# pycompression/python-zlib-ng

Hardware: AMD Instinct MI355X
Metric: MB/s compress+decompress, 128 KiB blocks level 6 (higher is better)
Workload: dtype u8

## Files before the change

### python-zlib-ng_amd/csrc/zng_amd.hip

```cpp
#include "za_deflate.hip"
#include "za_inflate.hip"
#include "za_inflate_units.hip"
#include "za_inflate_spans.hip"
#include "za_bgzf.hip"
#include "za_grep.hip"
#include "za_grep_records.hip"
#include "za_tabix.hip"
#include "za_faidx.hip"
#include "za_batch.hip"
#include "za_dict.hip"
#include "za_checksum.hip"
#include "../../include/zng_amd.h"

#include <algorithm>
#include <chrono>
#include <cstdio>
#include <cstdlib>
#include <cstring>
#include <mutex>
#include <string>
#include <thread>
#include <vector>

static_assert(sizeof(zngamd_member) == sizeof(ZaMember), "member layout");
static_assert(sizeof(zngamd_span) == sizeof(ZaSpan) && ZNGAMD_SPAN_PAD == ZA_SPAN_PAD && ZNGAMD_SPAN_CRC == ZA_SPAN_CRC, "span layout");
static_assert(sizeof(zngamd_batch_item) == sizeof(ZaBatchItem) && sizeof(zngamd_batch_result) == sizeof(ZaBatchResult) &&
              ZNGAMD_BATCH_PAD == ZA_BATCH_PAD && ZNGAMD_BATCH_TABLE == ZA_BATCH_TABLE && ZNGAMD_BATCH_OUTFULL == ZA_BATCH_OUTFULL, "batch layout");
static_assert(ZNGAMD_ZDICT_MISMATCH == ZA_ZDICT_MISMATCH, "zdict status");
static_assert(sizeof(zngamd_bgzf_block) == sizeof(ZaBgzfBlock) && sizeof(zngamd_bgzf_slice) == sizeof(ZaBgzfSlice) && ZNGAMD_BGZF_MAX_INPUT == ZA_BGZF_MAX_IN &&
              ZNGAMD_BGZF_SLICE_BLOCK == ZA_SLICE_BLOCK && ZNGAMD_BGZF_SLICE_TABLE == ZA_SLICE_TABLE, "bgzf layout");
static_assert(sizeof(zngamd_bgzf_count_row) == sizeof(ZaBgzfCount) && sizeof(zngamd_bgzf_pos) == sizeof(ZaBgzfPos) && sizeof(zngamd_bgzf_line_range) == 2 * sizeof(ZaBgzfPos) &&
              ZNGAMD_BGZF_SLICE_RANK == ZA_SLICE_RANK && ZNGAMD_BGZF_RANK_END == ZA_RANK_END && ZNGAMD_BGZF_COUNT_LAST == ZA_COUNT_LAST, "bgzf line layout");
static_assert(sizeof(zngamd_bgzf_pattern) == sizeof(ZaGrepPat) && sizeof(zngamd_bgzf_grep_row) == sizeof(ZaGrepRow) && sizeof(ZaGrepRow) == sizeof(ZaBgzfSlice) &&
              sizeof(zngamd_bgzf_grep_totals) == 40 && offsetof(ZaGrepTotals, covered) == offsetof(zngamd_bgzf_grep_totals, covered) && sizeof(ZaGrepTotals) <= 64 &&
              ZNGAMD_BGZF_GREP_INVERT == ZA_GREP_INVERT && ZNGAMD_BGZF_GREP_LINE_START == ZA_GREP_LINE_START && ZNGAMD_BGZF_GREP_FINAL == ZA_GREP_FINAL &&
              ZNGAMD_BGZF_GREP_COUNT_ONLY == ZA_GREP_COUNT_ONLY && ZNGAMD_BGZF_GREP_MAX_PATTERNS == ZA_GREP_MAX_PAT && ZNGAMD_BGZF_GREP_MAX_PATTERN == ZA_GREP_MAX_LEN,
              "bgzf grep layout");
static_assert(sizeof(zngamd_bgzf_grep_records_totals) == sizeof(ZaGrepRecTotals) && sizeof(ZaGrepRecTotals) == 64 &&
              offsetof(ZaGrepRecTotals, covered) == offsetof(zngamd_bgzf_grep_records_totals, covered) && sizeof(ZaGrepTotals) == 56 &&
              ZNGAMD_BGZF_GREP_MAX_RECORD_LINES == ZA_GREP_REC_MAX, "bgzf grep records layout");
static_assert(sizeof(zngamd_tabix_conf) == sizeof(ZaTbxConf) && sizeof(zngamd_tabix_name) == sizeof(ZaTbxName) && sizeof(zngamd_tabix_bin) == sizeof(ZaTbxBin) &&
              sizeof(zngamd_tabix_win) == sizeof(ZaTbxWin) && sizeof(zngamd_tabix_region) == sizeof(ZaTbxRegion) && sizeof(zngamd_tabix_span) == sizeof(ZaTbxSpan) &&
              sizeof(zngamd_tabix_row) == sizeof(ZaTbxRow) && sizeof(zngamd_bgzf_tabix_totals) == 104 && sizeof(ZaTbxState) <= 64 &&
              ZNGAMD_BGZF_TABIX_FINAL == ZA_TBX_FINAL && ZNGAMD_BGZF_FETCH_COUNT_ONLY == ZA_TBX_COUNT_ONLY && ZNGAMD_TABIX_MAX_POS == ZA_TBX_MAX_POS, "bgzf tabix layout");
static_assert(sizeof(zngamd_faidx_carry) == sizeof(ZaFaiCarry) && sizeof(ZaFaiCarry) == 32 && sizeof(zngamd_faidx_row) == sizeof(ZaFaiRow) && sizeof(ZaFaiRow) == 48 &&
              sizeof(zngamd_faidx_span) == sizeof(ZaFaiSpan) && sizeof(ZaFaiSpan) == 40 && sizeof(zngamd_bgzf_faidx_totals) == 104 && sizeof(ZaFaiState) == 88 &&
              ZNGAMD_BGZF_FAIDX_FINAL == ZA_FAI_FINAL && ZNGAMD_FAIDX_SPAN_RC == ZA_FAI_RC && ZNGAMD_FAIDX_MAX_SPAN == ZA_FAI_MAX_SPAN &&
              ZNGAMD_BGZF_SLICE_STALE == ZA_SLICE_STALE && ZNGAMD_FAIDX_OPEN == ZA_FAI_OPEN && ZNGAMD_FAIDX_GAP == ZA_FAI_GAP, "bgzf faidx layout");
static_assert(ZNGAMD_SLOT_STRIDE % 4 == 0 && ZNGAMD_SLOT_STRIDE >= ZA_MAX_UNIT + 32, "slot stride");
static_assert(ZNGAMD_UNIT_MAX == ZA_MAX_UNIT && ZNGAMD_SEG == ZA_SEG, "constants");

#define ZA_CH_STREAMS_PER_CU (ZA_HASH_BITS >= 14 ? 2u : 3u)
static const ZaLevel ZA_LEVELS[10] = {
    {0, 0, ZA_WIN, 0, 0, 0, 0, 0, 3, 0},
    {1, 16, ZA_WIN, 16, 0, 0, 256, 4096, 3, 0}, {2, 16, ZA_WIN, 16, 0, 0, 256, 4096, 3, 0}, {3, 16, ZA_WIN, 16, 0, 0, 256, 4096, 3, 0},
    {2, 16, ZA_WIN, 16, 0, 1, 4096, 32768, 3, 0}, {2, 16, ZA_WIN, 16, 1, 1, 4096, 32768, 3, 0}, {3, 16, ZA_WIN, 16, 1, 1, 4096, 32768, 3, 0},
    {4, 32, ZA_WIN, 258, 1, 1, 4096, 32768, 3, 0}, {8, 64, ZA_WIN, 258, 1, 1, 4096, 32768, 3, 0}, {12, 128, ZA_WIN, 258, 1, 1, 4096, 32768, 3, 0}};

template <typename T> struct DevBuf {
    T *p = nullptr; size_t cap = 0;
    hipError_t ensure(size_t n)
    {
        if (n <= cap) return hipSuccess;
        if (p) { (void)hipFree(p); p = nullptr; cap = 0; }
        size_t want = n * sizeof(T) >= ((size_t)64 << 20) ? n + 64 : n + n / 8 + 64;
        hipError_t e = hipMalloc((void **)&p, want * sizeof(T));
        if (e != hipSuccess) { want = n; e = hipMalloc((void **)&p, want * sizeof(T)); }
        if (e == hipSuccess) cap = want;
        return e;
    }
    void release() { if (p) (void)hipFree(p); p = nullptr; cap = 0; }
};

struct EvPair { hipEvent_t a, b; int cls; };

static thread_local std::string za_tl_err;
struct ZaErrSlot {
    ZaErrSlot &operator=(const char *m) { za_tl_err = m; return *this; }
    ZaErrSlot &operator=(const std::string &m) { za_tl_err = m; return *this; }
    const char *c_str() const { return za_tl_err.c_str(); }
};

struct zngamd_ctx {
    int device = 0;
    hipStream_t own_stream = nullptr, stream = nullptr;
    ZaErrSlot err;
    std::mutex mu;
    uint32_t *d_crc_table = nullptr, *d_x8k = nullptr;
    uint32_t *d_crc_slice4 = nullptr;
    uint32_t chunk_units = 16384;
    DevBuf<uint16_t> links; DevBuf<uint32_t> best, tok, segtok, hist, codes; DevBuf<ZaPlan> plan;
    uint16_t *prev_p = nullptr, *linkb_p = nullptr, *linkc_p = nullptr; uint32_t *tok_p = nullptr;
    bool debug_keep = false, last_kept = false; DevBuf<uint32_t> best_keep, dpcost;
    std::vector<uint32_t> last_ulen_host; bool last_ulen_on_host = false;
    const uint32_t *last_unit_len = nullptr;
    DevBuf<ZaUnit> units; DevBuf<uint32_t> segbits, cidx, status, runs;
    uint32_t last_units = 0; bool last_single_chunk = false;
    std::vector<ZaUnit> last_hu;
    std::vector<ZaUnit> plan_in; std::vector<uint32_t> plan_runs; uint32_t plan_ch = 0;
    std::vector<zngamd_block> blocks_in; std::vector<ZaUnit> blocks_hu; uint64_t blocks_len = 0;
    uint32_t chain_slots = 512;
    uint32_t chain_run = 0;
    DevBuf<uint8_t> st_in, st_out, st_slots, st_aux, hdr; DevBuf<uint32_t> st_len, st_crc; DevBuf<uint64_t> st_off;
    DevBuf<uint64_t> ccand, csurv; DevBuf<ZaChunkRes> cres; DevBuf<ZaChunk> cchunks; DevBuf<uint16_t> out16, ccomp; DevBuf<uint8_t> winbuf;
    DevBuf<uint16_t> uarea; uint32_t uarea_marked = 0;
    DevBuf<ZaCkPart> ck; DevBuf<uint32_t> matchq; DevBuf<ZaCand> cands; DevBuf<ZaMember> members; DevBuf<int32_t> mstatus;
    void *d_small = nullptr;
    uint64_t paths[4] = {0, 0, 0, 0};
    uint64_t indexed_units = 0;
    uint64_t span_stats[2] = {0, 0};
    DevBuf<uint8_t> sp_in, sp_win, sp_out; DevBuf<ZaSpan> sp_tab; DevBuf<int32_t> sp_status;
    DevBuf<uint8_t> bt_out, bt_out2, bt_def; DevBuf<ZaBatchItem> bt_items, bt_items2; DevBuf<ZaBatchResult> bt_res, bt_res2;
    DevBuf<uint32_t> bt_first, bt_ulen, bt_ucrc; DevBuf<uint64_t> bt_uoff, bt_total;
    DevBuf<uint8_t> bt_dict, bt_prime;
    DevBuf<uint8_t> dt_data, dt_dict; DevBuf<uint32_t> dt_hash, dt_freq; DevBuf<uint16_t> dt_shadow;
    DevBuf<ZaBatchItem> dt_items; DevBuf<ZaDictBest> dt_best; DevBuf<ZaDictState> dt_state;
    DevBuf<uint32_t> bg_len; DevBuf<ZaBgzfBlock> bg_table; DevBuf<ZaBgzfSlice> bg_slices; DevBuf<int32_t> bg_sstat; DevBuf<uint8_t> bg_out;
    uint64_t bgzf_stats[3] = {0, 0, 0};
    DevBuf<ZaBgzfCount> bg_rows; DevBuf<ZaBgzfPos> bg_q; DevBuf<uint64_t> bg_pos; DevBuf<int32_t> bg_pstat, bg_pre; DevBuf<uint32_t> bg_rlen;
    DevBuf<uint8_t> gp_par; DevBuf<ulonglong2> gp_bits; DevBuf<ZaGrepTile> gp_tiles; DevBuf<ZaGrepCarry> gp_carry; DevBuf<ZaGrepRow> gp_rows; DevBuf<uint32_t> gp_lens;
    DevBuf<unsigned long long> tb_bits, tb_data, tb_name, tb_bin, tb_key, tb_raise, tb_blk, tb_tot; DevBuf<uint32_t> tb_tcnt, tb_di, tb_lens; DevBuf<uint64_t> tb_tbase;
    DevBuf<ZaTbxLine> tb_lines; DevBuf<ZaTbxName> tb_names; DevBuf<ZaTbxBin> tb_bins; DevBuf<ZaTbxWin> tb_wins;
    DevBuf<uint8_t> tb_par; DevBuf<ZaTbxSpan> tb_spans; DevBuf<ZaTbxRow> tb_rows; DevBuf<uint32_t> tb_srows; DevBuf<int32_t> tb_sstat; DevBuf<uint64_t> tb_sbase;
    std::vector<uint8_t> tb_host;
    DevBuf<unsigned long long> fa_x, fa_bw; DevBuf<uint64_t> fa_start; DevBuf<uint32_t> fa_hline, fa_first, fa_last; DevBuf<ZaFaiRow> fa_rows; DevBuf<ZaFaiSpan> fa_spans;
    DevBuf<unsigned long long> gr_start, gr_sel, gr_len; DevBuf<uint8_t> gr_hit;
    std::vector<uint8_t> gp_host;
    uint8_t *h_stage = nullptr; size_t h_stage_cap = 0;
    uint8_t *h_up = nullptr; size_t h_up_cap = 0;
    uint8_t *h_tab = nullptr; size_t h_tab_cap = 0;
    hipEvent_t ev_up = nullptr, ev_tab = nullptr; bool up_busy = false, tab_busy = false;
    hipEvent_t ev_copy[2] = {nullptr, nullptr};
    bool prof = false; std::vector<EvPair> evs; std::vector<hipEvent_t> pool;
    double ms[ZNGAMD_K_COUNT] = {0}; uint64_t launches[ZNGAMD_K_COUNT] = {0};
};

#define HIPCHK(ctx, call) do { hipError_t e_ = (call); if (e_ != hipSuccess) { \
    (ctx)->err = std::string(#call) + ": " + hipGetErrorString(e_); return ZNGAMD_E_HIP; } } while (0)

static int fail(zngamd_ctx *c, int code, const char *msg) { c->err = msg; return code; }
#define ZA_ABI_GUARD catch (const std::bad_alloc &) { return ZNGAMD_MEM_ERROR; } catch (...) { return ZNGAMD_E_ARG; }


static bool trace_on() { static const bool on = getenv("ZNGAMD_TRACE") != nullptr; return on; }
struct PhaseClock {
    zngamd_ctx *c; const char *name; std::chrono::steady_clock::time_point t;
    PhaseClock(zngamd_ctx *c_, const char *n) : c(c_), name(n) { if (trace_on()) t = std::chrono::steady_clock::now(); }
    ~PhaseClock()
    {
        if (!trace_on()) return;
        if (c) (void)hipStreamSynchronize(c->stream);
        fprintf(stderr, "zng_amd trace: %-34s %9.3f ms\n", name, std::chrono::duration<double, std::milli>(std::chrono::steady_clock::now() - t).count());
    }
};

static hipEvent_t ev_get(zngamd_ctx *c)
{
    if (!c->pool.empty()) { hipEvent_t e = c->pool.back(); c->pool.pop_back(); return e; }
    hipEvent_t e; (void)hipEventCreate(&e); return e;
}
struct ProfScope {
    zngamd_ctx *c; int cls; hipEvent_t a = nullptr;
    ProfScope(zngamd_ctx *c_, int cls_) : c(c_), cls(cls_) { if (c->prof) { a = ev_get(c); (void)hipEventRecord(a, c->stream); } }
    ~ProfScope() { if (c->prof) { hipEvent_t b = ev_get(c); (void)hipEventRecord(b, c->stream); c->evs.push_back({a, b, cls}); } }
};
static void prof_collect(zngamd_ctx *c)
{
    for (auto &e : c->evs) {
        float t = 0; (void)hipEventSynchronize(e.b);
        if (hipEventElapsedTime(&t, e.a, e.b) == hipSuccess) { c->ms[e.cls] += t; c->launches[e.cls]++; }
        c->pool.push_back(e.a); c->pool.push_back(e.b);
    }
    c->evs.clear();
}

extern "C" {

const char *zngamd_version(void) { return "zng_amd 0.6 (gfx950)"; }
int zngamd_abi(void) { return ZNGAMD_ABI; }
int zngamd_kernel_class_count(void) { return ZNGAMD_K_COUNT; }

int zngamd_device_count(void)
try {
    int n = 0;
    if (hipGetDeviceCount(&n) != hipSuccess) return 0;
    return n;
} ZA_ABI_GUARD

int zngamd_ctx_create(int device, zngamd_ctx **out)
try {
    if (!out) return ZNGAMD_E_ARG;
    *out = nullptr;
    int n = 0;
    if (hipGetDeviceCount(&n) != hipSuccess || n <= 0 || device < 0 || device >= n) return ZNGAMD_E_HIP;
    if (hipSetDevice(device) != hipSuccess) return ZNGAMD_E_HIP;
    zngamd_ctx *c = new zngamd_ctx();
    c->device = device;
    if (hipStreamCreateWithFlags(&c->own_stream, hipStreamNonBlocking) != hipSuccess) { delete c; return ZNGAMD_E_HIP; }
    c->stream = c->own_stream;
    if (const char *e = getenv("ZNGAMD_CHUNK_UNITS")) { long v = atol(e); if (v >= 1 && v <= (1 << 20)) c->chunk_units = (uint32_t)v; }
    if (const char *e = getenv("ZNGAMD_CHAIN_RUN")) { long v = atol(e); if (v >= 1 && v <= (1 << 20)) c->chain_run = (uint32_t)v; }
    { int cus = 0; if (hipDeviceGetAttribute(&cus, hipDeviceAttributeMultiprocessorCount, device) == hipSuccess && cus > 0) c->chain_slots = (uint32_t)cus * ZA_CH_STREAMS_PER_CU; }
    uint32_t tab[256], x8k[64];
    for (uint32_t i = 0; i < 256; i++) { uint32_t v = i; for (int k = 0; k < 8; k++) v = (v & 1) ? (0xEDB88320u ^ (v >> 1)) : (v >> 1); tab[i] = v; }
    {
        uint32_t xs = 0x80000000u, sq = 0x00800000u;
        for (int i = 0; i < 11; i++) sq = za_multmodp(sq, sq);
        for (int k = 0; k < 64; k++) { x8k[k] = xs; xs = za_multmodp(xs, sq); }
    }
    if (hipMalloc((void **)&c->d_crc_table, sizeof tab) != hipSuccess || hipMalloc((void **)&c->d_x8k, sizeof x8k) != hipSuccess ||
        hipMalloc(&c->d_small, 256) != hipSuccess ||
        hipMemcpy(c->d_crc_table, tab, sizeof tab, hipMemcpyHostToDevice) != hipSuccess ||
        hipMemcpy(c->d_x8k, x8k, sizeof x8k, hipMemcpyHostToDevice) != hipSuccess) {
        zngamd_ctx_destroy(c); return ZNGAMD_E_HIP;
    }
    {
        std::vector<uint32_t> s4(ZA_CK_TABS);
        for (int i = 0; i < 256; i++) s4[i] = tab[i];
        for (int t = 1; t < 4; t++) for (int i = 0; i < 256; i++) s4[256 * t + i] = (s4[256 * (t - 1) + i] >> 8) ^ tab[s4[256 * (t - 1) + i] & 0xFF];
        uint32_t x32 = 0x00800000u;
        for (int i = 0; i < 5; i++) x32 = za_multmodp(x32, x32);
        uint32_t xs = 0x80000000u;
        for (int k = 0; k < 128; k++) { s4[1152 + k] = xs; xs = za_multmodp(xs, x32); }
        const uint32_t x2016 = s4[1152 + 63];
        for (int k = 0; k < 8; k++) for (uint32_t v = 0; v < 16; v++) s4[1024 + 16 * k + v] = za_multmodp(x2016, v << (4 * k));
        {
            uint32_t xt = 0x80000000u;
            for (int t = 0; t <= 512; t++) { s4[ZA_CK_XT + t] = xt; xt = za_multmodp(xt, 0x00800000u); }
            for (int j = 0; j < 4; j++) {
                const uint32_t step = s4[ZA_CK_XT + (64 << j)];
                uint32_t xk = 0x80000000u;
                for (int k = 0; k < 256; k++) { s4[ZA_CK_XS + 256 * j + k] = xk; xk = za_multmodp(xk, step); }
            }
        }
        if (hipMalloc((void **)&c->d_crc_slice4, s4.size() * 4) != hipSuccess ||
            hipMemcpy(c->d_crc_slice4, s4.data(), s4.size() * 4, hipMemcpyHostToDevice) != hipSuccess) {
            zngamd_ctx_destroy(c); return ZNGAMD_E_HIP;
        }
    }
    *out = c;
    return ZNGAMD_OK;
} ZA_ABI_GUARD

void zngamd_ctx_destroy(zngamd_ctx *c)
{
    if (!c) return;
    (void)hipSetDevice(c->device);
    if (c->stream) (void)hipStreamSynchronize(c->stream);
    prof_collect(c);
    for (auto e : c->pool) (void)hipEventDestroy(e);
    c->links.release(); c->best_keep.release(); c->dpcost.release(); c->hdr.release(); c->best.release(); c->tok.release(); c->segtok.release(); c->hist.release(); c->codes.release();
    c->plan.release(); c->units.release(); c->segbits.release(); c->cidx.release(); c->status.release();
    c->st_in.release(); c->st_out.release(); c->st_slots.release(); c->st_aux.release(); c->st_len.release(); c->st_crc.release();
    c->ccand.release(); c->csurv.release(); c->cres.release(); c->cchunks.release(); c->out16.release(); c->ccomp.release(); c->winbuf.release(); c->uarea.release();
    c->st_off.release(); c->runs.release(); c->ck.release(); c->matchq.release(); c->cands.release(); c->members.release(); c->mstatus.release();
    c->sp_in.release(); c->sp_win.release(); c->sp_out.release(); c->sp_tab.release(); c->sp_status.release();
    c->bt_out.release(); c->bt_out2.release(); c->bt_def.release(); c->bt_items.release(); c->bt_items2.release(); c->bt_res.release(); c->bt_res2.release();
    c->bt_first.release(); c->bt_ulen.release(); c->bt_ucrc.release(); c->bt_uoff.release(); c->bt_total.release();
    c->bt_dict.release(); c->bt_prime.release();
    c->dt_data.release(); c->dt_dict.release(); c->dt_hash.release(); c->dt_freq.release(); c->dt_shadow.release();
    c->dt_items.release(); c->dt_best.release(); c->dt_state.release();
    c->bg_len.release(); c->bg_table.release(); c->bg_slices.release(); c->bg_sstat.release(); c->bg_out.release();
    c->bg_rows.release(); c->bg_q.release(); c->bg_pos.release(); c->bg_pstat.release(); c->bg_pre.release(); c->bg_rlen.release();
    c->tb_bits.release(); c->tb_data.release(); c->tb_name.release(); c->tb_bin.release(); c->tb_key.release(); c->tb_raise.release(); c->tb_blk.release();
    c->tb_tot.release(); c->tb_tcnt.release(); c->tb_di.release(); c->tb_lens.release(); c->tb_tbase.release(); c->tb_lines.release(); c->tb_names.release();
    c->tb_bins.release(); c->tb_wins.release(); c->tb_par.release(); c->tb_spans.release(); c->tb_rows.release(); c->tb_srows.release(); c->tb_sstat.release(); c->tb_sbase.release();
    c->fa_x.release(); c->fa_bw.release(); c->fa_start.release(); c->fa_hline.release(); c->fa_first.release(); c->fa_last.release(); c->fa_rows.release(); c->fa_spans.release();
    c->gp_par.release(); c->gp_bits.release(); c->gp_tiles.release(); c->gp_carry.release(); c->gp_rows.release(); c->gp_lens.release();
    c->gr_start.release(); c->gr_sel.release(); c->gr_len.release(); c->gr_hit.release();
    if (c->h_stage) (void)hipHostFree(c->h_stage);
    if (c->h_up) (void)hipHostFree(c->h_up);
    if (c->h_tab) (void)hipHostFree(c->h_tab);
    if (c->ev_up) (void)hipEventDestroy(c->ev_up);
    if (c->ev_tab) (void)hipEventDestroy(c->ev_tab);
    for (auto &e : c->ev_copy) if (e) (void)hipEventDestroy(e);
    if (c->d_crc_table) (void)hipFree(c->d_crc_table);
    if (c->d_x8k) (void)hipFree(c->d_x8k);
    if (c->d_crc_slice4) (void)hipFree(c->d_crc_slice4);
    if (c->d_small) (void)hipFree(c->d_small);
    if (c->own_stream) (void)hipStreamDestroy(c->own_stream);
    delete c;
}

const char *zngamd_last_error(zngamd_ctx *c) { return c ? c->err.c_str() : "no context"; }

int zngamd_set_stream(zngamd_ctx *c, void *s)
try {
    if (!c) return ZNGAMD_E_ARG;
    (void)hipStreamSynchronize(c->stream);
    c->stream = s ? (hipStream_t)s : c->own_stream;
    return ZNGAMD_OK;
} ZA_ABI_GUARD

int zngamd_sync(zngamd_ctx *c)
try {
    if (!c) return ZNGAMD_E_ARG;
    HIPCHK(c, hipStreamSynchronize(c->stream));
    prof_collect(c);
    return ZNGAMD_OK;
} ZA_ABI_GUARD

int zngamd_dmalloc(zngamd_ctx *c, size_t bytes, void **dptr)
try {
    if (!c || !dptr) return ZNGAMD_E_ARG;
    HIPCHK(c, hipSetDevice(c->device));
    HIPCHK(c, hipMalloc(dptr, bytes ? bytes : 1));
    return ZNGAMD_OK;
} ZA_ABI_GUARD
int zngamd_dfree(zngamd_ctx *c, void *dptr) { if (!c) return ZNGAMD_E_ARG; HIPCHK(c, hipFree(dptr)); return ZNGAMD_OK; }
int zngamd_h2d(zngamd_ctx *c, void *dst, const void *src, size_t bytes)
try {
    if (!c) return ZNGAMD_E_ARG;
    if (bytes) { HIPCHK(c, hipMemcpyAsync(dst, src, bytes, hipMemcpyHostToDevice, c->stream)); HIPCHK(c, hipStreamSynchronize(c->stream)); }
    return ZNGAMD_OK;
} ZA_ABI_GUARD

int zngamd_d2h(zngamd_ctx *c, void *dst, const void *src, size_t bytes)
try {
    if (!c) return ZNGAMD_E_ARG;
    if (bytes) { HIPCHK(c, hipMemcpyAsync(dst, src, bytes, hipMemcpyDeviceToHost, c->stream)); HIPCHK(c, hipStreamSynchronize(c->stream)); }
    return ZNGAMD_OK;
} ZA_ABI_GUARD

int zngamd_d2d(zngamd_ctx *c, void *dst, const void *src, size_t bytes)
try {
    if (!c) return ZNGAMD_E_ARG;
    HIPCHK(c, hipSetDevice(c->device));
    if (bytes) HIPCHK(c, hipMemcpyAsync(dst, src, bytes, hipMemcpyDeviceToDevice, c->stream));
    return ZNGAMD_OK;
} ZA_ABI_GUARD

int zngamd_dmemset(zngamd_ctx *c, void *dst, int value, size_t bytes)
try {
    if (!c) return ZNGAMD_E_ARG;
    HIPCHK(c, hipSetDevice(c->device));
    if (bytes) HIPCHK(c, hipMemsetAsync(dst, value, bytes, c->stream));
    return ZNGAMD_OK;
} ZA_ABI_GUARD

int zngamd_mem_info(zngamd_ctx *c, uint64_t *free_bytes, uint64_t *total_bytes)
try {
    if (!c || !free_bytes || !total_bytes) return ZNGAMD_E_ARG;
    HIPCHK(c, hipSetDevice(c->device));
    size_t f = 0, t = 0;
    HIPCHK(c, hipMemGetInfo(&f, &t));
    *free_bytes = f; *total_bytes = t;
    return ZNGAMD_OK;
} ZA_ABI_GUARD

int zngamd_decode_paths(zngamd_ctx *c, uint64_t *members, int reset)
try {
    if (!c || !members) return ZNGAMD_E_ARG;
    std::lock_guard<std::mutex> g(c->mu);
    for (int i = 0; i < ZNGAMD_PATH_COUNT; i++) { members[i] = c->paths[i]; if (reset) c->paths[i] = 0; }
    return ZNGAMD_OK;
// ... 49 lines not shown
        for (uint64_t k = ZA_MAX_UNIT; k; k >>= 1) { if (k & 1) xp = za_multmodp(sq, xp); sq = za_multmodp(sq, sq); }
        for (uint64_t i = 0; i < nspan; i++) {
            if (parts[i].len == ZA_MAX_UNIT) crc = za_multmodp(xp, crc) ^ parts[i].crc;
            else crc = zngamd_crc32_combine(crc, parts[i].crc, parts[i].len);
        }
        *crc_io = crc;
    }
    if (adler_io) {
        uint64_t A = *adler_io & 0xFFFF, B = (*adler_io >> 16) & 0xFFFF;
        for (uint64_t i = 0; i < nspan; i++) {
            B = (B + (uint64_t)(parts[i].len % 65521u) * A + parts[i].b) % 65521u;
            A = (A + parts[i].a) % 65521u;
        }
        *adler_io = (uint32_t)((B << 16) | A);
    }
}

static int checksum_dev(zngamd_ctx *c, const uint8_t *d, uint64_t n, uint32_t *crc_io, uint32_t *adler_io)
{
    if (n == 0) return ZNGAMD_OK;
    PhaseClock pc(c, "checksum of a device buffer");
    std::vector<ZaCkPart> parts;
    const int r = checksum_launch(c, d, n, crc_io != nullptr, adler_io != nullptr, parts);
    if (r) return r;
    HIPCHK(c, hipStreamSynchronize(c->stream));
    checksum_fold(parts, crc_io, adler_io);
    return ZNGAMD_OK;
}

static int pinned_ensure(zngamd_ctx *c, uint8_t **p, size_t *cap, size_t bytes)
{
    if (bytes <= *cap) return ZNGAMD_OK;
    if (*p) (void)hipHostFree(*p);
    *p = nullptr; *cap = 0;
    const size_t want = bytes + bytes / 4 + 4096;
    HIPCHK(c, hipHostMalloc((void **)p, want, hipHostMallocDefault));
    *cap = want;
    return ZNGAMD_OK;
}

#define ZNGAMD_SMALL_UP (1u << 20)
static int stage_in(zngamd_ctx *c, const uint8_t *in, uint64_t n, uint64_t pad_front = 0)
{
    PhaseClock pc(c, "stage_in (host -> device)");
    HIPCHK(c, hipSetDevice(c->device));
    HIPCHK(c, c->st_in.ensure(pad_front + n + 64));
    if (n <= ZNGAMD_SMALL_UP) {
        if (!c->ev_up) HIPCHK(c, hipEventCreateWithFlags(&c->ev_up, hipEventDisableTiming));
        if (c->up_busy) { HIPCHK(c, hipEventSynchronize(c->ev_up)); c->up_busy = false; }
        const int r = pinned_ensure(c, &c->h_up, &c->h_up_cap, n + 64);
        if (r) return r;
        if (n) memcpy(c->h_up, in, n);
        memset(c->h_up + n, 0, 64);
        HIPCHK(c, hipMemcpyAsync(c->st_in.p + pad_front, c->h_up, n + 64, hipMemcpyHostToDevice, c->stream));
        HIPCHK(c, hipEventRecord(c->ev_up, c->stream));
        c->up_busy = true;
        return ZNGAMD_OK;
    }
    if (n) HIPCHK(c, hipMemcpyAsync(c->st_in.p + pad_front, in, n, hipMemcpyHostToDevice, c->stream));
    HIPCHK(c, hipMemsetAsync(c->st_in.p + pad_front + n, 0, 64, c->stream));
    return ZNGAMD_OK;
}

int zngamd_crc32_dev(zngamd_ctx *c, uint32_t crc, const void *dbuf, size_t len, uint32_t *out)
try {
    if (!c || !out) return ZNGAMD_E_ARG;
    std::lock_guard<std::mutex> g(c->mu);
    HIPCHK(c, hipSetDevice(c->device));
    uint32_t v = crc;
    int r = checksum_dev(c, (const uint8_t *)dbuf, len, &v, nullptr);
    *out = v;
    return r;
} ZA_ABI_GUARD

int zngamd_crc32(zngamd_ctx *c, uint32_t crc, const uint8_t *buf, size_t len, uint32_t *out)
try {
    if (!c || !out || (!buf && len)) return ZNGAMD_E_ARG;
    std::lock_guard<std::mutex> g(c->mu);
    int r = stage_in(c, buf, len);
    if (r) return r;
    uint32_t v = crc;
    r = checksum_dev(c, c->st_in.p, len, &v, nullptr);
    *out = v;
    return r;
} ZA_ABI_GUARD

int zngamd_adler32(zngamd_ctx *c, uint32_t adler, const uint8_t *buf, size_t len, uint32_t *out)
try {
    if (!c || !out || (!buf && len)) return ZNGAMD_E_ARG;
    std::lock_guard<std::mutex> g(c->mu);
    int r = stage_in(c, buf, len);
    if (r) return r;
    uint32_t v = ((((adler >> 16) & 0xFFFFu) % 65521u) << 16) | ((adler & 0xFFFFu) % 65521u);
    r = checksum_dev(c, c->st_in.p, len, nullptr, &v);
    *out = v;
    return r;
} ZA_ABI_GUARD

int zngamd_level_ok(int level) { return level >= -1 && level <= 9; }

static int strategy_of(const zngamd_block *blocks, uint32_t n_blocks) { return n_blocks ? ZNGAMD_STRATEGY_OF(blocks[0].flags) : ZNGAMD_STRATEGY_DEFAULT; }

static uint32_t unit_size_of(const zngamd_block &b) { return (b.flags & ZNGAMD_FLAG_UNITS16K) ? ZA_SMALL_UNIT : (uint32_t)ZA_MAX_UNIT; }
static uint32_t units_of(const zngamd_block &b) { const uint64_t U = unit_size_of(b); return b.len == 0 ? 1u : (uint32_t)(((uint64_t)b.len + U - 1) / U); }

uint32_t zngamd_count_units(const zngamd_block *blocks, uint32_t n_blocks)
{
    uint64_t t = 0;
    for (uint32_t i = 0; i < n_blocks; i++) t += units_of(blocks[i]);
    return t > 0xFFFFFFFFull ? 0xFFFFFFFFu : (uint32_t)t;
}

static int build_units(zngamd_ctx *c, const zngamd_block *blocks, uint32_t n_blocks, uint64_t in_len, std::vector<ZaUnit> &hu)
{
    hu.clear();
    for (uint32_t b = 0; b < n_blocks; b++) {
        const zngamd_block &B = blocks[b];
        if (B.dict_len > ZA_WIN || B.dict_len > B.off || B.off + B.len > in_len) return fail(c, ZNGAMD_E_ARG, "block outside the input buffer");
        const uint32_t nu = units_of(B);
        const uint64_t U = unit_size_of(B);
        for (uint32_t k = 0; k < nu; k++) {
            ZaUnit u;
            const uint64_t rel = (uint64_t)k * U;
            u.in_off = B.off + rel;
            u.in_len = (uint32_t)std::min<uint64_t>(U, B.len - rel);
            u.dict_len = (uint32_t)std::min<uint64_t>(ZA_WIN, (uint64_t)B.dict_len + rel);
            u.flags = (B.flags & (ZNGAMD_FLAG_FLATHDR | ZNGAMD_FLAG_SEG2K)) | ((k == nu - 1) ? (B.flags & ZNGAMD_FLAG_FINAL) : 0u);
            u.flags |= (uint32_t)za_seg_shift_for(u.in_len, u.flags) << 8;
            u.block = b;
            if (!hu.empty()) {
                const ZaUnit &pv = hu.back();
                if (u.dict_len == ZA_WIN && pv.in_len >= ZA_WIN && (pv.in_len & 3u) == 0u && pv.in_off + pv.in_len == u.in_off) u.flags |= ZA_FLAG_CARRY;
            }
            hu.push_back(u);
        }
    }
    return ZNGAMD_OK;
}

struct PackedDst { uint8_t *d_dst = nullptr; uint64_t cap = 0; uint64_t *d_unit_off = nullptr;
                   uint64_t *d_total = nullptr; uint32_t *d_status = nullptr; };
static int deflate_units_dev(zngamd_ctx *c, const uint8_t *d_in, uint64_t in_len, const std::vector<ZaUnit> &hu, int level,
                             uint8_t *d_slots, uint32_t *d_unit_len, uint32_t *d_unit_crc, int max_dist = ZA_WIN,
                             const PackedDst *packed = nullptr, int strategy = ZNGAMD_STRATEGY_DEFAULT)
{
    if (level == -1) level = 6;
    if (level < 0 || level > 9) return fail(c, ZNGAMD_STREAM_ERROR, "Bad compression level");
    if (strategy < ZNGAMD_STRATEGY_DEFAULT || strategy > ZNGAMD_STRATEGY_FIXED) return fail(c, ZNGAMD_STREAM_ERROR, "Bad compression strategy");
    const bool runs_only = level > 0 && (strategy == ZNGAMD_STRATEGY_HUFFMAN_ONLY || strategy == ZNGAMD_STRATEGY_RLE);
    const bool search = level > 0 && !runs_only;
    const uint32_t n = (uint32_t)hu.size();
    if (n == 0) return ZNGAMD_OK;
    HIPCHK(c, hipSetDevice(c->device));
    uint32_t ch = std::min(n, c->chunk_units);
    const size_t ntab = ZA_LEVELS[level].use_c ? 3 : 2;
    if (search) {
        const size_t held = c->links.cap * 2 + c->best.cap * 4 + c->tok.cap * 4 + c->best_keep.cap * 4;
        size_t free_b = 0, total_b = 0;
        if (ch > 64 && hipMemGetInfo(&free_b, &total_b) == hipSuccess) {
            auto need = [&](uint32_t k) { return (size_t)k * (ntab * ZA_PREV_STRIDE * 2 + ZA_BEST_STRIDE * 4 + (c->debug_keep ? (ZA_BEST_STRIDE + ZA_TOK_STRIDE) * 4 : 0) + 8192); };
            while (ch > 64 && need(ch) > held && need(ch) - held > free_b - free_b / 16) ch = (ch + 1) / 2;
        }
    }
    HIPCHK(c, c->units.ensure(n)); HIPCHK(c, c->segbits.ensure((size_t)n * ZA_SEGB_STRIDE)); HIPCHK(c, c->cidx.ensure((size_t)n * ZA_CIDX_STRIDE)); HIPCHK(c, c->status.ensure(n));
    if (runs_only) {
        const size_t held = c->links.cap * 2 + (c->debug_keep ? c->tok.cap * 4 : 0);
        size_t free_b = 0, total_b = 0;
        if (ch > 64 && hipMemGetInfo(&free_b, &total_b) == hipSuccess) {
            auto need = [&](uint32_t k) { return (size_t)k * (ZA_TOK_STRIDE * 4 + 8192); };
            while (ch > 64 && need(ch) > held && need(ch) - held > free_b - free_b / 16) ch = (ch + 1) / 2;
        }
        if (c->debug_keep) { HIPCHK(c, c->tok.ensure((size_t)ch * ZA_TOK_STRIDE)); c->tok_p = c->tok.p; }
        else { HIPCHK(c, c->links.ensure((size_t)ch * ZA_TOK_STRIDE * 2)); c->tok_p = (uint32_t *)c->links.p; }
    }
    if (search) {
        const size_t tab = (size_t)ch * ZA_PREV_STRIDE + 8;
        HIPCHK(c, c->links.ensure(ntab * tab)); HIPCHK(c, c->best.ensure((size_t)ch * ZA_BEST_STRIDE));
        c->prev_p = c->links.p; c->linkb_p = c->links.p + tab; c->linkc_p = ntab > 2 ? c->links.p + 2 * tab : nullptr;
        if (ZA_LEVELS[level].dp) HIPCHK(c, c->dpcost.ensure((size_t)ch * ZA_DP_COSTS));
        if (c->debug_keep) {
            HIPCHK(c, c->best_keep.ensure((size_t)ch * ZA_BEST_STRIDE));
            HIPCHK(c, c->tok.ensure((size_t)ch * ZA_TOK_STRIDE));
            c->tok_p = c->tok.p;
        } else {
            static_assert(2 * ZA_PREV_STRIDE * 2 >= ZA_TOK_STRIDE * 4, "token words fit two link tables");
            c->tok_p = (uint32_t *)c->links.p;
        }
    }
    HIPCHK(c, c->segtok.ensure((size_t)ch * ZA_MAX_SEGS)); HIPCHK(c, c->hist.ensure((size_t)ch * ZA_HIST_STRIDE));
    HIPCHK(c, c->codes.ensure((size_t)ch * ZA_CODE_STRIDE)); HIPCHK(c, c->plan.ensure(ch));
    uint64_t *d_run_total = (uint64_t *)((uint8_t *)c->d_small + 224);
    uint64_t *d_offs = nullptr;
    if (packed) {
        HIPCHK(c, c->hdr.ensure((size_t)ch * ZA_HDR_STRIDE));
        d_offs = packed->d_unit_off;
        if (!d_offs) { HIPCHK(c, c->st_off.ensure(n)); d_offs = c->st_off.p; }
        if (packed->d_total) d_run_total = packed->d_total;
    }
    uint32_t *d_status = (packed && packed->d_status) ? packed->d_status : c->status.p;
    const bool same_plan = c->plan_ch == ch && c->plan_in.size() == hu.size() && c->last_hu.size() == hu.size() &&
                           memcmp(c->plan_in.data(), hu.data(), hu.size() * sizeof(ZaUnit)) == 0;
    if (!same_plan) {
        c->plan_in.clear(); c->plan_ch = 0; c->last_hu.clear();
        std::vector<ZaUnit> hv(hu);
        std::vector<uint32_t> run_start;
        for (uint32_t c0 = 0; c0 < n; c0 += ch) {
            const uint32_t m = std::min(ch, n - c0);
            const uint32_t L = c->chain_run ? c->chain_run : std::min<uint32_t>(8u, std::max<uint32_t>(1u, m / (2u * c->chain_slots)));
            const uint32_t Ls = c->chain_run ? c->chain_run : std::max<uint32_t>(1u, L / 4u);
            const uint32_t big_end = c->chain_run ? m : (uint32_t)((uint64_t)m * 4 / 5 / L * L);
            uint32_t next_cut = 0;
            for (uint32_t i = 0; i < m; i++) {
                ZaUnit &u = hv[c0 + i];
                const bool cut = i == next_cut || !(u.flags & ZA_FLAG_CARRY);
                if (cut) { u.flags |= ZA_FLAG_RUNHEAD; run_start.push_back(i); next_cut = i + (i < big_end ? L : Ls); }
            }
            run_start.push_back(m);
        }
        HIPCHK(c, c->runs.ensure(run_start.size()));
        if (n <= 4096) {
            const size_t rb = run_start.size() * 4, ub = (size_t)n * sizeof(ZaUnit);
            if (!c->ev_tab) HIPCHK(c, hipEventCreateWithFlags(&c->ev_tab, hipEventDisableTiming));
            if (c->tab_busy) { HIPCHK(c, hipEventSynchronize(c->ev_tab)); c->tab_busy = false; }
            const int rp = pinned_ensure(c, &c->h_tab, &c->h_tab_cap, rb + ub);
            if (rp) return rp;
            memcpy(c->h_tab, hv.data(), ub);
            memcpy(c->h_tab + ub, run_start.data(), rb);
            HIPCHK(c, hipMemcpyAsync(c->units.p, c->h_tab, ub, hipMemcpyHostToDevice, c->stream));
            HIPCHK(c, hipMemcpyAsync(c->runs.p, c->h_tab + ub, rb, hipMemcpyHostToDevice, c->stream));
            HIPCHK(c, hipEventRecord(c->ev_tab, c->stream));
            c->tab_busy = true;
        } else {
        HIPCHK(c, hipMemcpyAsync(c->runs.p, run_start.data(), run_start.size() * 4, hipMemcpyHostToDevice, c->stream));
        HIPCHK(c, hipMemcpyAsync(c->units.p, hv.data(), (size_t)n * sizeof(ZaUnit), hipMemcpyHostToDevice, c->stream));
        HIPCHK(c, hipStreamSynchronize(c->stream));
        }
        c->last_hu.swap(hv);
        c->plan_runs.swap(run_start);
        c->plan_in = hu; c->plan_ch = ch;
    }
    const std::vector<uint32_t> &run_start = c->plan_runs;
    ZaLevel L = ZA_LEVELS[level];
    L.max_dist = (max_dist < 1 || max_dist > ZA_WIN) ? ZA_WIN : max_dist;
    if (strategy == ZNGAMD_STRATEGY_FILTERED) L.min_len = 6;
    const int fixed_only = strategy == ZNGAMD_STRATEGY_FIXED ? 1 : 0;
    L.fixed_cost = fixed_only;
    size_t run_pos = 0;
    for (uint32_t c0 = 0; c0 < n; c0 += ch) {
        const uint32_t m = std::min(ch, n - c0);
        const ZaUnit *du = c->units.p + c0;
        uint32_t nruns = 0;
        while (run_start[run_pos + nruns] != m) nruns++;
        const uint32_t *d_runs = c->runs.p + run_pos;
        run_pos += nruns + 1;
        if (runs_only) {
            ProfScope ps(c, ZNGAMD_K_PARSE);
            if (strategy == ZNGAMD_STRATEGY_RLE)
                hipLaunchKernelGGL(za_k_parse_rle<true>, dim3(m), dim3(64), 0, c->stream, d_in, du, c->tok_p, c->segtok.p, c->hist.p,
                                   d_unit_crc + c0, c->d_crc_table, c->d_x8k);
            else
                hipLaunchKernelGGL(za_k_parse_rle<false>, dim3(m), dim3(64), 0, c->stream, d_in, du, c->tok_p, c->segtok.p, c->hist.p,
                                   d_unit_crc + c0, c->d_crc_table, c->d_x8k);
        } else if (search) {
            { ProfScope ps(c, ZNGAMD_K_CHAINS);
              hipLaunchKernelGGL(za_k_chains<ZA_TABLE_A>, dim3(nruns), dim3(256), 0, c->stream, d_in, du, d_runs, c->prev_p, L.dp ? c->dpcost.p : (uint32_t *)nullptr);
              hipLaunchKernelGGL(za_k_chains<ZA_TABLE_B>, dim3(nruns), dim3(256), 0, c->stream, d_in, du, d_runs, c->linkb_p, (uint32_t *)nullptr);
              if (L.use_c) hipLaunchKernelGGL(za_k_chains<ZA_TABLE_C>, dim3(nruns), dim3(256), 0, c->stream, d_in, du, d_runs, c->linkc_p, (uint32_t *)nullptr); }
            { ProfScope ps(c, ZNGAMD_K_SEARCH);
#define ZA_LAUNCH_SEARCH(...) hipLaunchKernelGGL((za_k_search<__VA_ARGS__>), dim3(nruns), dim3(ZA_SEARCH_THREADS), 0, c->stream, d_in, in_len, du, d_runs, \
                                                 c->prev_p, c->linkb_p, L.use_c ? c->linkc_p : c->linkb_p, c->best.p, c->dpcost.p, L)
              if (L.cap > 16) { if (L.use_c) ZA_LAUNCH_SEARCH(true, 0, true); else ZA_LAUNCH_SEARCH(true, 0, false); }
              else if (L.chain == 1) { if (L.use_c) ZA_LAUNCH_SEARCH(false, 1, true); else ZA_LAUNCH_SEARCH(false, 1, false); }
              else if (L.chain == 2) { if (L.use_c) ZA_LAUNCH_SEARCH(false, 2, true); else ZA_LAUNCH_SEARCH(false, 2, false); }
              else if (L.chain == 3) { if (L.use_c) ZA_LAUNCH_SEARCH(false, 3, true); else ZA_LAUNCH_SEARCH(false, 3, false); }
              else { if (L.use_c) ZA_LAUNCH_SEARCH(false, 0, true); else ZA_LAUNCH_SEARCH(false, 0, false); }
#undef ZA_LAUNCH_SEARCH
            }
            if (L.dp) {
                if (c->debug_keep) HIPCHK(c, hipMemcpyAsync(c->best_keep.p, c->best.p, (size_t)m * ZA_BEST_STRIDE * 4, hipMemcpyDeviceToDevice, c->stream));
                ProfScope ps(c, ZNGAMD_K_OPTPARSE);
                if (L.cap > 16 || !ZA_STATS_FOLD) hipLaunchKernelGGL(za_k_dpstats, dim3(m), dim3(256), 0, c->stream, du, c->best.p, c->dpcost.p);
                hipLaunchKernelGGL(za_k_optparse, dim3(m), dim3(64), 0, c->stream, du, c->best.p, c->dpcost.p, c->tok_p, L);
            }
            { ProfScope ps(c, ZNGAMD_K_PARSE);
              if (L.min_len > ZA_MIN_MATCH)
                  hipLaunchKernelGGL(za_k_parse<true>, dim3(m), dim3(64), 0, c->stream, du, c->best.p, c->tok_p, c->segtok.p, c->hist.p,
                                     d_unit_crc + c0, c->d_crc_table, c->d_x8k, L);
              else
                  hipLaunchKernelGGL(za_k_parse<false>, dim3(m), dim3(64), 0, c->stream, du, c->best.p, c->tok_p, c->segtok.p, c->hist.p,
                                     d_unit_crc + c0, c->d_crc_table, c->d_x8k, L); }
        } else {
            ProfScope ps(c, ZNGAMD_K_PARSE);
            hipLaunchKernelGGL(za_k_unit_crc, dim3(m), dim3(64), 0, c->stream, d_in, du, d_unit_crc + c0, c->d_crc_table, c->d_x8k);
        }
        if (packed) {
            { ProfScope ps(c, ZNGAMD_K_PLAN);
              hipLaunchKernelGGL(za_k_plan, dim3(m), dim3(64), 0, c->stream, du, c->hist.p, c->codes.p, c->plan.p,
                                 (uint8_t *)nullptr, 0u, level, c->hdr.p, d_unit_len + c0, fixed_only); }
            { ProfScope ps(c, ZNGAMD_K_GATHER);
              hipLaunchKernelGGL(za_k_offsets, dim3(1), dim3(m <= 64 ? 64 : 1024), 0, c->stream, d_unit_len + c0, m, 0u, 0ull, d_offs + c0, d_run_total,
                                 (const ZaUnit *)nullptr, c0 ? (const uint64_t *)d_run_total : (const uint64_t *)nullptr, 1); }
            { ProfScope ps(c, ZNGAMD_K_PACK);
              hipLaunchKernelGGL(za_k_pack, dim3(m), dim3(64), 0, c->stream, d_in, du, c->tok_p, c->segtok.p, c->codes.p, c->plan.p,
                                 c->segbits.p + (size_t)c0 * ZA_SEGB_STRIDE, c->cidx.p + (size_t)c0 * ZA_CIDX_STRIDE, packed->d_dst,
                                 0u, d_unit_len + c0, d_status + c0, (const uint64_t *)(d_offs + c0), packed->cap, (const uint8_t *)c->hdr.p); }
        } else {
        { ProfScope ps(c, ZNGAMD_K_PLAN);
          hipLaunchKernelGGL(za_k_plan, dim3(m), dim3(64), 0, c->stream, du, c->hist.p, c->codes.p, c->plan.p,
                             d_slots + (size_t)c0 * ZNGAMD_SLOT_STRIDE, (uint32_t)ZNGAMD_SLOT_STRIDE, level, (uint8_t *)nullptr, (uint32_t *)nullptr, fixed_only); }
        { ProfScope ps(c, ZNGAMD_K_PACK);
          hipLaunchKernelGGL(za_k_pack, dim3(m), dim3(64), 0, c->stream, d_in, du, c->tok_p, c->segtok.p, c->codes.p, c->plan.p,
                             c->segbits.p + (size_t)c0 * ZA_SEGB_STRIDE, c->cidx.p + (size_t)c0 * ZA_CIDX_STRIDE, d_slots + (size_t)c0 * ZNGAMD_SLOT_STRIDE,
                             (uint32_t)ZNGAMD_SLOT_STRIDE, d_unit_len + c0, c->status.p + c0, (const uint64_t *)nullptr, 0ull, (const uint8_t *)nullptr); }
        }
        HIPCHK(c, hipGetLastError());
    }
    c->last_units = n; c->last_single_chunk = (n <= ch); c->last_kept = c->debug_keep; c->last_unit_len = d_unit_len; c->last_ulen_on_host = false;
    return ZNGAMD_OK;
}

int zngamd_deflate_blocks_dev(zngamd_ctx *c, const void *d_in, uint64_t in_len, const zngamd_block *blocks, uint32_t n_blocks,
                              int level, void *d_slots, uint32_t *d_unit_len, uint32_t *d_unit_crc, uint32_t *h_unit_block)
try {
    if (!c || (!blocks && n_blocks) || !d_slots || !d_unit_len || !d_unit_crc) return ZNGAMD_E_ARG;
    std::lock_guard<std::mutex> g(c->mu);
    int r = ZNGAMD_OK;
    if (!(n_blocks && c->blocks_in.size() == n_blocks && c->blocks_len == in_len &&
          memcmp(c->blocks_in.data(), blocks, (size_t)n_blocks * sizeof(zngamd_block)) == 0)) {
        c->blocks_in.clear();
        r = build_units(c, blocks, n_blocks, in_len, c->blocks_hu);
        if (r) return r;
        c->blocks_in.assign(blocks, blocks + n_blocks); c->blocks_len = in_len;
    }
    const std::vector<ZaUnit> &hu = c->blocks_hu;
    if (h_unit_block) for (size_t i = 0; i < hu.size(); i++) h_unit_block[i] = hu[i].block;
    r = deflate_units_dev(c, (const uint8_t *)d_in, in_len, hu, level, (uint8_t *)d_slots, d_unit_len, d_unit_crc, ZA_WIN, nullptr,
                          strategy_of(blocks, n_blocks));
    if (r) return r;
    HIPCHK(c, hipStreamSynchronize(c->stream));
    prof_collect(c);
    return ZNGAMD_OK;
} ZA_ABI_GUARD

int zngamd_deflate_blocks_packed_dev(zngamd_ctx *c, const void *d_in, uint64_t in_len, const zngamd_block *blocks, uint32_t n_blocks,
                                     int level, void *d_out, uint64_t out_cap, uint32_t *d_unit_len, uint32_t *d_unit_crc,
                                     uint64_t *d_unit_off, uint64_t *total_bytes)
try {
    if (!c || (!blocks && n_blocks) || !d_out || !d_unit_len || !d_unit_crc || !total_bytes) return ZNGAMD_E_ARG;
    std::lock_guard<std::mutex> g(c->mu);
    int r = ZNGAMD_OK;
    if (!(n_blocks && c->blocks_in.size() == n_blocks && c->blocks_len == in_len &&
          memcmp(c->blocks_in.data(), blocks, (size_t)n_blocks * sizeof(zngamd_block)) == 0)) {
        c->blocks_in.clear();
        r = build_units(c, blocks, n_blocks, in_len, c->blocks_hu);
        if (r) return r;
        c->blocks_in.assign(blocks, blocks + n_blocks); c->blocks_len = in_len;
    }
    const std::vector<ZaUnit> &hu = c->blocks_hu;
    *total_bytes = 0;
    if (hu.empty()) return ZNGAMD_OK;
    PackedDst pd; pd.d_dst = (uint8_t *)d_out; pd.cap = out_cap; pd.d_unit_off = d_unit_off;
    r = deflate_units_dev(c, (const uint8_t *)d_in, in_len, hu, level, nullptr, d_unit_len, d_unit_crc, ZA_WIN, &pd, strategy_of(blocks, n_blocks));
    if (r) return r;
    const uint64_t *d_run_total = (const uint64_t *)((const uint8_t *)c->d_small + 224);
    std::vector<uint32_t> st(hu.size());
    HIPCHK(c, hipMemcpyAsync(total_bytes, d_run_total, 8, hipMemcpyDeviceToHost, c->stream));
    HIPCHK(c, hipMemcpyAsync(st.data(), c->status.p, st.size() * 4ull, hipMemcpyDeviceToHost, c->stream));
    HIPCHK(c, hipStreamSynchronize(c->stream));
// ... 3596 lines not shown
```

Measured before the change: 56730.

## Size chunks by free memory share and taper chain run lengths by slot count

```diff
diff --git a/python-zlib-ng_amd/csrc/zng_amd.hip b/python-zlib-ng_amd/csrc/zng_amd.hip
--- a/python-zlib-ng_amd/csrc/zng_amd.hip
+++ b/python-zlib-ng_amd/csrc/zng_amd.hip
@@ -51,6 +51,7 @@
 static_assert(ZNGAMD_UNIT_MAX == ZA_MAX_UNIT && ZNGAMD_SEG == ZA_SEG, "constants");
 
 #define ZA_CH_STREAMS_PER_CU (ZA_HASH_BITS >= 14 ? 2u : 3u)
+#define ZA_WS_SHARE_DIV 4u
 static const ZaLevel ZA_LEVELS[10] = {
     {0, 0, ZA_WIN, 0, 0, 0, 0, 0, 3, 0},
     {1, 16, ZA_WIN, 16, 0, 0, 256, 4096, 3, 0}, {2, 16, ZA_WIN, 16, 0, 0, 256, 4096, 3, 0}, {3, 16, ZA_WIN, 16, 0, 0, 256, 4096, 3, 0},
@@ -88,7 +89,7 @@
     std::mutex mu;
     uint32_t *d_crc_table = nullptr, *d_x8k = nullptr;
     uint32_t *d_crc_slice4 = nullptr;
-    uint32_t chunk_units = 16384;
+    uint32_t chunk_units = 0;
     DevBuf<uint16_t> links; DevBuf<uint32_t> best, tok, segtok, hist, codes; DevBuf<ZaPlan> plan;
     uint16_t *prev_p = nullptr, *linkb_p = nullptr, *linkc_p = nullptr; uint32_t *tok_p = nullptr;
     bool debug_keep = false, last_kept = false; DevBuf<uint32_t> best_keep, dpcost;
@@ -100,6 +101,7 @@
     std::vector<ZaUnit> plan_in; std::vector<uint32_t> plan_runs; uint32_t plan_ch = 0;
     std::vector<zngamd_block> blocks_in; std::vector<ZaUnit> blocks_hu; uint64_t blocks_len = 0;
     uint32_t chain_slots = 512;
+    uint32_t search_slots = 256;
     uint32_t chain_run = 0;
     DevBuf<uint8_t> st_in, st_out, st_slots, st_aux, hdr; DevBuf<uint32_t> st_len, st_crc; DevBuf<uint64_t> st_off;
     DevBuf<uint64_t> ccand, csurv; DevBuf<ZaChunkRes> cres; DevBuf<ZaChunk> cchunks; DevBuf<uint16_t> out16, ccomp; DevBuf<uint8_t> winbuf;
@@ -200,7 +202,8 @@
     c->stream = c->own_stream;
     if (const char *e = getenv("ZNGAMD_CHUNK_UNITS")) { long v = atol(e); if (v >= 1 && v <= (1 << 20)) c->chunk_units = (uint32_t)v; }
     if (const char *e = getenv("ZNGAMD_CHAIN_RUN")) { long v = atol(e); if (v >= 1 && v <= (1 << 20)) c->chain_run = (uint32_t)v; }
-    { int cus = 0; if (hipDeviceGetAttribute(&cus, hipDeviceAttributeMultiprocessorCount, device) == hipSuccess && cus > 0) c->chain_slots = (uint32_t)cus * ZA_CH_STREAMS_PER_CU; }
+    { int cus = 0; if (hipDeviceGetAttribute(&cus, hipDeviceAttributeMultiprocessorCount, device) == hipSuccess && cus > 0) { c->chain_slots = (uint32_t)cus * ZA_CH_STREAMS_PER_CU; c->search_slots = (uint32_t)cus; } }
+    if (const char *e = getenv("ZNGAMD_CHAIN_SLOTS")) { long v = atol(e); if (v >= 1 && v <= (1 << 20)) { c->chain_slots = (uint32_t)v; c->search_slots = std::max<uint32_t>(1u, (uint32_t)v / ZA_CH_STREAMS_PER_CU); } }
     uint32_t tab[256], x8k[64];
     for (uint32_t i = 0; i < 256; i++) { uint32_t v = i; for (int k = 0; k < 8; k++) v = (v & 1) ? (0xEDB88320u ^ (v >> 1)) : (v >> 1); tab[i] = v; }
     {
@@ -556,24 +559,21 @@
     const uint32_t n = (uint32_t)hu.size();
     if (n == 0) return ZNGAMD_OK;
     HIPCHK(c, hipSetDevice(c->device));
-    uint32_t ch = std::min(n, c->chunk_units);
+    uint32_t ch = c->chunk_units ? std::min(n, c->chunk_units) : n;
     const size_t ntab = ZA_LEVELS[level].use_c ? 3 : 2;
-    if (search) {
-        const size_t held = c->links.cap * 2 + c->best.cap * 4 + c->tok.cap * 4 + c->best_keep.cap * 4;
+    auto fit_set = [&](size_t per_unit, size_t held) {
         size_t free_b = 0, total_b = 0;
-        if (ch > 64 && hipMemGetInfo(&free_b, &total_b) == hipSuccess) {
-            auto need = [&](uint32_t k) { return (size_t)k * (ntab * ZA_PREV_STRIDE * 2 + ZA_BEST_STRIDE * 4 + (c->debug_keep ? (ZA_BEST_STRIDE + ZA_TOK_STRIDE) * 4 : 0) + 8192); };
-            while (ch > 64 && need(ch) > held && need(ch) - held > free_b - free_b / 16) ch = (ch + 1) / 2;
-        }
-    }
+        if (ch <= 64 || hipMemGetInfo(&free_b, &total_b) != hipSuccess) return;
+        auto need = [&](uint32_t k) { return (size_t)k * per_unit; };
+        while (ch > 64 && need(ch) > held && need(ch) - held > free_b - free_b / 16) ch = (ch + 1) / 2;
+        if (!c->chunk_units) while (ch > 64 && need(ch) > (free_b + held) / ZA_WS_SHARE_DIV) ch = (ch + 1) / 2;
+    };
+    if (search)
+        fit_set(ntab * ZA_PREV_STRIDE * 2 + ZA_BEST_STRIDE * 4 + (c->debug_keep ? (ZA_BEST_STRIDE + ZA_TOK_STRIDE) * 4 : 0) + 8192,
+                c->links.cap * 2 + c->best.cap * 4 + c->tok.cap * 4 + c->best_keep.cap * 4);
     HIPCHK(c, c->units.ensure(n)); HIPCHK(c, c->segbits.ensure((size_t)n * ZA_SEGB_STRIDE)); HIPCHK(c, c->cidx.ensure((size_t)n * ZA_CIDX_STRIDE)); HIPCHK(c, c->status.ensure(n));
     if (runs_only) {
-        const size_t held = c->links.cap * 2 + (c->debug_keep ? c->tok.cap * 4 : 0);
-        size_t free_b = 0, total_b = 0;
-        if (ch > 64 && hipMemGetInfo(&free_b, &total_b) == hipSuccess) {
-            auto need = [&](uint32_t k) { return (size_t)k * (ZA_TOK_STRIDE * 4 + 8192); };
-            while (ch > 64 && need(ch) > held && need(ch) - held > free_b - free_b / 16) ch = (ch + 1) / 2;
-        }
+        fit_set(ZA_TOK_STRIDE * 4 + 8192, c->links.cap * 2 + (c->debug_keep ? c->tok.cap * 4 : 0));
         if (c->debug_keep) { HIPCHK(c, c->tok.ensure((size_t)ch * ZA_TOK_STRIDE)); c->tok_p = c->tok.p; }
         else { HIPCHK(c, c->links.ensure((size_t)ch * ZA_TOK_STRIDE * 2)); c->tok_p = (uint32_t *)c->links.p; }
     }
@@ -612,12 +612,15 @@
             const uint32_t m = std::min(ch, n - c0);
             const uint32_t L = c->chain_run ? c->chain_run : std::min<uint32_t>(8u, std::max<uint32_t>(1u, m / (2u * c->chain_slots)));
             const uint32_t Ls = c->chain_run ? c->chain_run : std::max<uint32_t>(1u, L / 4u);
-            const uint32_t big_end = c->chain_run ? m : (uint32_t)((uint64_t)m * 4 / 5 / L * L);
+            const uint64_t slots = std::max<uint32_t>(c->search_slots, (c->chain_slots + 1u) / 2u);
+            const uint32_t n_single = (c->chain_run || Ls == 1u) ? 0u : (uint32_t)std::min<uint64_t>(m, slots * Ls);
+            const uint32_t n_mid = c->chain_run ? 0u : (uint32_t)std::min<uint64_t>(m - n_single, slots * L);
+            const uint32_t big_end = (m - n_single - n_mid) / L * L, mid_end = m - n_single;
             uint32_t next_cut = 0;
             for (uint32_t i = 0; i < m; i++) {
                 ZaUnit &u = hv[c0 + i];
                 const bool cut = i == next_cut || !(u.flags & ZA_FLAG_CARRY);
-                if (cut) { u.flags |= ZA_FLAG_RUNHEAD; run_start.push_back(i); next_cut = i + (i < big_end ? L : Ls); }
+                if (cut) { u.flags |= ZA_FLAG_RUNHEAD; run_start.push_back(i); next_cut = i + (i < big_end ? L : i < mid_end ? Ls : 1u); }
             }
             run_start.push_back(m);
         }
```

Measured after the change: 58840, median of 6. +3.7%, better.
